# zhing2006/hala-renderer

Measured on AMD Instinct MI355X. Metric: Mrays/s, higher is better.
Workload: dtype f32

## Files before the change

hala-renderer_amd/csrc/renderer.hip:

```cpp
#include <hip/hip_runtime.h>

#include <algorithm>
#include <cmath>
#include <cstdio>
#include <cstring>
#include <memory>
#include <string>
#include <sys/stat.h>
#include <vector>

#include "adaptive.h"
#include "denoise.h"
#include "dyn_api.h"
#include "hala_types.h"
#include "host_image.h"
#include "host_scene.h"
#include "host_util.h"
#include "kernels.h"

namespace rt { std::string decode_image_file_rgba8(const char* path, uint32_t* w, uint32_t* h, std::vector<uint8_t>* rgba); }

using namespace rt;

namespace {
// ... 112 lines not shown
    std::vector<uint32_t> insts;
    DeviceArray<hala_gpu_mesh_data> d_md;
    DeviceArray<uint32_t> d_first, d_gid, d_inst;
    ~Blas() { if (b.topology) bvh_free_topology(b.topology); }
  };
  std::vector<std::unique_ptr<Blas>> blas;
  bool two_level = false;
  uint32_t instancing_mode = 0;
  std::vector<uint8_t> inst_instanced;
  std::vector<int32_t> prim_blas;
  uint32_t tlas_capacity = 0, tlas_nodes = 0, stored_tris = 0;
  std::vector<InstRef> inst_refs;
  DeviceArray<InstRef> d_inst_refs;
  DeviceArray<InstInfo> d_inst_info;
  DeviceArray<Tri> d_tris_by_id, d_tris;
  DeviceArray<Tri> d_tris_any;
  DeviceArray<ShadeTri> d_shade_tris;
  DeviceArray<BvhNode4> d_nodes;
  uint32_t lds_nodes = 0, lds_tris = 0;
  bool staged = false;
  uint32_t leaf_max_built = 0;
  float ray_eps = 0.0f;
  DeviceArray<uint2> d_spill;
  LaunchCfg lcfg{};
  uint32_t fuse_mode = 1;

  bool has_env = false;
  uint32_t env_w = 0, env_h = 0;
  DeviceArray<float4> d_env;
  DeviceArray<float> d_env_total, d_marginal, d_conditional;
  float env_total_sum = 0.0f;

  uint32_t real_pixels = 0;
  uint32_t rank = 0, world = 1, tile_size = 32, tiles_x = 0, tiles_y = 0, tiles_per_rank = 0, perm_a_inv = 0, perm_b = 7;
  uint32_t slot_count = 0;
  uint32_t blocks_x = 0;
  size_t image_pixels() const { return world <= 1 ? (size_t)width * height : (size_t)slot_count; }
  uint32_t batch_capacity = 1;

  DeviceArray<float4> img_local[4];
  DeviceArray<float4> img_full[4];
  bool full_valid[4] = {false, false, false, false};
  DenoiseBuffers denoise;
  bool denoised = false;
  AdaptiveState adaptive;
  DeviceArray<P3> ps_lr, ps_le, ps_alb, ps_nrm;
  DeviceArray<hala_ray> q_rays[2];
  DeviceArray<float4> q_state[2];
  DeviceArray<hala_hit> q_hits;
  DeviceArray<uint32_t> q_perm;
  DeviceArray<ShadowEntry> q_shadow[2];
  DeviceArray<Control> d_ctl;
  DeviceArray<WorkCounters> d_batch_work;

  uint64_t total_frames = 0;
  bool counting = false;
  hala_global_uniform last_uniform{};
  TraceEvents ring[kStatRing];
  int ring_pos = 0;
  bool vertices_dirty = false;
  bool materials_dirty_any = false;
  bool materials_dirty_any_refit = false;
  bool any_invisible = false;
  bool any_translucent = false;
  DeviceArray<uint8_t> d_material_any_class;
  std::vector<uint8_t> material_any_class;
  uint32_t launch_event_period = 0;
  unsigned long long update_counter = 0;
  hala_rt_statistics stats{};
  hipEvent_t scratch_event = nullptr;
  hipStream_t scratch_stream = nullptr;
  hipEvent_t batch_done = nullptr;
  ncclComm_t comm = nullptr;
  bool comm_owned = false;
  int comm_rank = 0, comm_world = 1;
  hipStream_t gather_stream = nullptr;
  DeviceArray<float4> gather_stage[4], gather_recv[4];
  hipEvent_t ev_rendered = nullptr, ev_staged = nullptr, ev_gathered = nullptr;
  uint32_t gather_pending = 0;
  int scratch_acquire(hipStream_t s) {
    if (scratch_event && scratch_stream != s) RT_HIP(hipStreamWaitEvent(s, scratch_event, 0));
    return HALA_OK;
  }

  ~hala_rt_renderer() {
    if (device >= 0) (void)hipSetDevice(device);
    if (stream) (void)hipStreamSynchronize(stream);
    for (auto& t : ring) {
      for (auto e : t.ev) (void)hipEventDestroy(e);
      if (t.frame_begin) (void)hipEventDestroy(t.frame_begin);
      if (t.frame_end) (void)hipEventDestroy(t.frame_end);
      if (t.host_totals) (void)hipHostFree(t.host_totals);
      if (t.host_sizes) (void)hipHostFree(t.host_sizes);
    }
    if (batch_done) (void)hipEventDestroy(batch_done);
    if (gather_stream) { (void)hipStreamSynchronize(gather_stream); (void)hipStreamDestroy(gather_stream); }
    for (hipEvent_t e : {ev_rendered, ev_staged, ev_gathered}) if (e) (void)hipEventDestroy(e);
    if (comm && comm_owned) { if (const RcclApi* api = rccl_api(nullptr)) (void)api->CommDestroy(comm); }
    for (auto& i : img_local) i.release();
    for (auto& i : img_full) i.release();
    if (bvh.topology) bvh_free_topology(bvh.topology);
    blas.clear();
    if (stream) (void)hipStreamDestroy(stream);
  }

  SceneView view() const {
    SceneView sv{};
    sv.nodes = d_nodes.ptr; sv.tris = d_tris.ptr; sv.tris_any = any_invisible ? d_tris_any.ptr : d_tris.ptr; sv.tris_by_id = d_tris_by_id.ptr; sv.shade_tris = d_shade_tris.ptr;
    sv.inst_first_tri = d_inst_first_tri.ptr; sv.primitives = d_instances.ptr; sv.materials = d_materials.ptr; sv.material_kind = d_material_kind.ptr;
    sv.lights = d_lights.ptr; sv.cameras = d_cameras.ptr;
    sv.textures = d_textures.ptr; sv.tex_arena = d_tex_arena.ptr; sv.tex_arena8 = d_tex_arena8.ptr; sv.tex_lut = d_srgb_lut.ptr; sv.texture_count = (uint32_t)host_textures.size(); sv.shade_sort = shade_sort ? 1u : 0u; sv.simple_materials = simple_materials ? 1u : 0u; sv.scatter_media = scatter_media ? 1u : 0u; sv.any_translucent = any_translucent ? 1u : 0u;
    sv.env_pixels = reinterpret_cast<const float*>(d_env.ptr); sv.env_marginal = d_marginal.ptr; sv.env_conditional = d_conditional.ptr;
    sv.node_count = bvh.node_count; sv.tri_count = bvh.tri_count; sv.lds_nodes = lds_nodes; sv.lds_tris = lds_tris;
    sv.inst_refs = d_inst_refs.ptr; sv.inst_info = d_inst_info.ptr; sv.instance_count = (uint32_t)hs.instances.size(); sv.two_level = two_level ? 1u : 0u;
    sv.ray_eps = ray_eps;
    sv.staged = staged ? 1u : 0u;
    return sv;
  }
  Queues queues() const {
    Queues q{};
    q.rays[0] = q_rays[0].ptr; q.rays[1] = q_rays[1].ptr; q.state[0] = q_state[0].ptr; q.state[1] = q_state[1].ptr;
    q.hits = q_hits.ptr; q.perm = q_perm.ptr; q.shadow[0] = q_shadow[0].ptr; q.shadow[1] = q_shadow[1].ptr;
    return q;
  }
  PathState path_state() const { return PathState{ps_lr.ptr, ps_le.ptr, ps_alb.ptr, ps_nrm.ptr}; }

  FrameConst frame_const(const hala_global_uniform& u, uint32_t samples = 1) const {
    FrameConst fc{};
    fc.u = u;
    fc.aspect = u.resolution[0] / u.resolution[1];
    float sn = 0.0f, cs = 1.0f;
    if (!hs.cameras.empty()) h_sincos_rad(0.5f * hs.cameras[0].yfov, &sn, &cs);
    fc.tan_half = sn / cs;
    fc.pixel_spread = 2.0f * fc.tan_half / u.resolution[1];
    fc.width = width; fc.height = height;
    fc.tile_size = tile_size; fc.tiles_x = tiles_x; fc.tiles_y = tiles_y; fc.world = world; fc.rank = rank; fc.blocks_x = blocks_x;
    fc.tiles_per_rank = tiles_per_rank; fc.perm_a = perm_a_inv; fc.perm_b = perm_b;
    fc.pixel_slots = slot_count; fc.samples = samples; fc.slot_count = slot_count * samples;
    if (adaptive.enabled) {
      fc.block_list = adaptive.lists[adaptive.cur].ptr;
      fc.pixel_slots = adaptive.active_blocks * kPixelBlock * kPixelBlock;
      fc.slot_count = fc.pixel_slots * samples;
    }
    return fc;
  }

  void reset_accumulation() {
    total_frames = 0;
    for (bool& v : full_valid) v = false;
    adaptive.restart(width * height);
  }
  uint32_t rendered_frames() const { return (uint32_t)std::min(total_frames, max_frames); }

  void resolve_slot(TraceEvents& t) {
    if (!t.pending) return;
    (void)hipEventSynchronize(t.frame_end);
    float ms = 0.0f;
    if (hipEventElapsedTime(&ms, t.frame_begin, t.frame_end) == hipSuccess) { stats.last_gpu_ms = ms; stats.gpu_ms_total += ms; }
    double tr[3] = {0.0, 0.0, 0.0}, sh = 0.0;
    unsigned long long rays[3] = {0, 0, 0}, launches[3] = {0, 0, 0};
    const QueueSizes* qs = t.host_sizes;
    for (size_t k = 0, depth = 0; k + 3 < t.used; k += 4, ++depth) {
      float m = 0.0f;
      const bool own_closest = depth == 0 || !((t.traced_mask >> depth) & 1ull);
      if (own_closest && hipEventElapsedTime(&m, t.ev[k], t.ev[k + 1]) == hipSuccess) {
        const unsigned long long n = depth == 0 ? (unsigned long long)t.primary_pixels * t.samples : qs->n_active[depth];
        tr[0] += m; rays[0] += n; launches[0] += 1;
        if (depth == 0) { stats.traverse_primary_ms_total += m; stats.traverse_primary_launches += 1; stats.rays_primary_timed += n; }
      }
      if (hipEventElapsedTime(&m, t.ev[k + 1], t.ev[k + 2]) == hipSuccess) sh += m;
      if (hipEventElapsedTime(&m, t.ev[k + 2], t.ev[k + 3]) == hipSuccess) {
        const unsigned long long ns = (unsigned long long)qs->n_shadow[0][depth] + qs->n_shadow[1][depth];
        if ((t.fused_mask >> depth) & 1ull) {
          tr[2] += m; launches[2] += 1;
          stats.rays_fused_shadow_timed += ns;
          if ((t.traced_mask >> (depth + 1)) & 1ull) stats.rays_fused_closest_timed += qs->n_active[depth + 1];
        } else { tr[1] += m; rays[1] += ns; }
      }
    }
    stats.traverse_ms_last_update = tr[0] + tr[1] + tr[2];
    stats.traverse_closest_ms_total += tr[0];
    stats.traverse_shadow_ms_total += tr[1];
    stats.traverse_fused_ms_total += tr[2];
    stats.shade_ms_total += sh;
    stats.traverse_closest_launches += launches[0];
    stats.traverse_fused_launches += launches[2];
    stats.shade_launches += t.used / 4;
    stats.traverse_shadow_launches += t.used ? t.shadow_launches : 0;
    stats.rays_closest_timed += rays[0]; stats.rays_shadow_timed += rays[1];
    stats.updates_rendered += t.samples;
    const Totals& tot = *t.host_totals;
    const unsigned long long rc = tot.rays_closest, rs = tot.rays_shadow;
    stats.rays_last_update = rc + rs;
    stats.rays_total += rc + rs;
    stats.rays_closest_total += rc;
    stats.rays_primary_total += (unsigned long long)t.primary_pixels * t.samples;
    stats.rays_shadow_total += rs;
    if (t.counted) {
      stats.nodes_closest_total += tot.steps[0][0]; stats.tris_closest_total += tot.steps[0][1];
      stats.nodes_shadow_total += tot.steps[1][0]; stats.tris_shadow_total += tot.steps[1][1];
      stats.rays_closest_counted += rc; stats.rays_shadow_counted += rs;
      stats.wave_steps_closest_total += tot.probe[0][0]; stats.leaf_passes_closest_total += tot.probe[0][1]; stats.leaf_lanes_closest_total += tot.probe[0][2];
      stats.nodes_primary_total += tot.primary_steps[0]; stats.tris_primary_total += tot.primary_steps[1];
      stats.rays_primary_counted += (unsigned long long)t.primary_pixels * t.samples;
      stats.wave_steps_shadow_total += tot.probe[1][0]; stats.leaf_passes_shadow_total += tot.probe[1][1]; stats.leaf_lanes_shadow_total += tot.probe[1][2];
    }
    t.pending = false;
  }
  hipEvent_t next_event(TraceEvents& t) {
    if (t.used == t.ev.size()) { hipEvent_t e = nullptr; (void)hipEventCreate(&e); t.ev.push_back(e); }
    return t.ev[t.used++];
  }
};

namespace {

int ensure_device(hala_rt_renderer* r) {
  if (!r) RT_FAIL("The renderer handle is null!");
  RT_HIP(hipSetDevice(r->device));
  return HALA_OK;
}

void compute_tiling(hala_rt_renderer* r) {
  if (r->world <= 1) {
    r->real_pixels = r->width * r->height;
    r->slot_count = r->real_pixels;
    r->blocks_x = 0;
    if (kPixelBlock) {
      r->blocks_x = (r->width + kPixelBlock - 1) / kPixelBlock;
      r->slot_count = r->blocks_x * ((r->height + kPixelBlock - 1) / kPixelBlock) * kPixelBlock * kPixelBlock;
    }
    r->tiles_x = r->tiles_y = r->tiles_per_rank = 0;
    return;
  }
  r->tiles_x = (r->width + r->tile_size - 1) / r->tile_size;
  r->tiles_y = (r->height + r->tile_size - 1) / r->tile_size;
  const uint32_t n = r->tiles_x * r->tiles_y;
  r->tiles_per_rank = (n + r->world - 1) / r->world;
  uint32_t A = 0x9E3779B1u % n;
  if (A == 0) A = 1;
  while (gcd_u32(A, n) != 1) ++A;
  r->perm_a_inv = mod_inverse(A, n);
  r->perm_b = 7;
  r->slot_count = r->tiles_per_rank * r->tile_size * r->tile_size;
  uint64_t real = 0;
  for (uint32_t t = 0; t < n; ++t) {
    const uint32_t k = (uint32_t)(((uint64_t)t * A + r->perm_b) % n);
    if (k % r->world != r->rank) continue;
    const uint32_t tx = t % r->tiles_x, ty = t / r->tiles_x;
    const uint32_t w = std::min(r->tile_size, r->width - tx * r->tile_size), h = std::min(r->tile_size, r->height - ty * r->tile_size);
    real += (uint64_t)w * h;
  }
  r->real_pixels = (uint32_t)real;
}

int alloc_wavefront(hala_rt_renderer* r, uint32_t samples) {
  const size_t n = (size_t)r->slot_count * samples;
  if (n > 0xfffffff0ull) RT_FAIL("The sample batch is too large for 32-bit path slots.");
  RT_HIP(r->ps_lr.resize(n)); RT_HIP(r->ps_le.resize(n)); RT_HIP(r->ps_alb.resize(n)); RT_HIP(r->ps_nrm.resize(n));
  RT_HIP(r->q_rays[0].resize(n)); RT_HIP(r->q_rays[1].resize(n)); RT_HIP(r->q_state[0].resize(n)); RT_HIP(r->q_state[1].resize(n));
  RT_HIP(r->q_hits.resize(n)); RT_HIP(r->q_perm.resize(n)); RT_HIP(r->q_shadow[0].resize(n)); RT_HIP(r->q_shadow[1].resize(n));
  r->batch_capacity = samples;
  return HALA_OK;
}

int alloc_frame_buffers(hala_rt_renderer* r) {
  const size_t n = r->slot_count;
  for (auto& i : r->img_local) { RT_HIP(i.resize(n)); RT_HIP(hipMemsetAsync(i.ptr, 0, n * sizeof(float4), r->stream)); }
  if (alloc_wavefront(r, 1) != HALA_OK) return HALA_ERR;
  RT_HIP(r->d_ctl.resize(1));
  RT_HIP(hipMemsetAsync(r->d_ctl.ptr, 0, sizeof(Control), r->stream));
  RT_HIP(r->d_batch_work.resize(1));
  return HALA_OK;
}

int upload_packed(hala_rt_renderer* r, bool geometry = true) {
  HostScene& hs = r->hs;
  if (geometry) {
  size_t nv = 0, ni = 0;
  r->prim_vertex_offset.clear(); r->prim_index_offset.clear();
  for (const auto& p : hs.prims) {
    r->prim_vertex_offset.push_back(nv); r->prim_index_offset.push_back(ni);
    nv += p.vertices.size();
    ni += (p.indices.size() + 3) & ~size_t(3);
  }
  RT_HIP(r->d_vertices.resize(nv)); RT_HIP(r->d_indices.resize(ni));
  for (size_t k = 0; k < hs.prims.size(); ++k) {
    const auto& p = hs.prims[k];
    if (!p.vertices.empty()) RT_HIP(hipMemcpyAsync(r->d_vertices.ptr + r->prim_vertex_offset[k], p.vertices.data(), p.vertices.size() * sizeof(hala_vertex), hipMemcpyHostToDevice, r->stream));
    if (!p.indices.empty()) RT_HIP(hipMemcpyAsync(r->d_indices.ptr + r->prim_index_offset[k], p.indices.data(), p.indices.size() * 4, hipMemcpyHostToDevice, r->stream));
  }
  }
  for (size_t i = 0; i < hs.instances.size(); ++i) {
    const uint32_t p = hs.instance_prim[i];
    hs.instances[i].vertices = reinterpret_cast<uint64_t>(r->d_vertices.ptr + r->prim_vertex_offset[p]);
    hs.instances[i].indices = reinterpret_cast<uint64_t>(r->d_indices.ptr + r->prim_index_offset[p]);
  }
  RT_HIP(r->d_cameras.upload(hs.cameras.data(), hs.cameras.size(), r->stream));
  RT_HIP(r->d_lights.upload(hs.lights.data(), hs.lights.size(), r->stream));
  RT_HIP(r->d_materials.upload(hs.gpu_materials.data(), hs.gpu_materials.size(), r->stream));
  {
    std::vector<uint8_t> kind(hs.gpu_materials.size());
    for (size_t i = 0; i < kind.size(); ++i) kind[i] = shade_kind_of(hs.gpu_materials[i], (uint32_t)hs.texture_image.size());
    RT_HIP(r->d_material_kind.upload(kind.data(), kind.size(), r->stream));
    r->material_kind = kind;
    uint32_t seen = 0;
    for (uint8_t k : kind) seen |= 1u << k;
    r->shade_sort = (seen & (seen - 1u)) != 0u;
    r->scatter_media = false;
    for (const auto& m : hs.gpu_materials) r->scatter_media = r->scatter_media || m.medium_type == 2u;
    r->simple_materials = seen == (1u << kShadeKindFirst);
  }
  RT_HIP(r->d_instances.upload(hs.instances.data(), hs.instances.size(), r->stream));
  RT_HIP(r->d_inst_first_tri.upload(hs.inst_first_tri.data(), hs.inst_first_tri.size(), r->stream));
  RT_HIP(hipStreamSynchronize(r->stream));
  return HALA_OK;
}

int upload_textures(hala_rt_renderer* r) {
  const HostScene& hs = r->hs;
  std::vector<TexDesc> img_desc(hs.images.size());
  size_t total_f = 0, total_8 = 0, largest_8 = 0;
  for (size_t k = 0; k < hs.images.size(); ++k) {
    TexDesc& td = img_desc[k];
    memset(&td, 0, sizeof(td));
    td.width = hs.images[k].width; td.height = hs.images[k].height; td.format = hs.images[k].format;
    uint32_t m = std::max(td.width, td.height), p2 = 1, lg = 0;
    while (p2 < m) { p2 <<= 1; ++lg; }
    td.mips = std::min<uint32_t>(lg + 1, kMaxMips);
    size_t& total = td.format == kTexFloat ? total_f : total_8;
    for (uint32_t l = 0; l < td.mips; ++l) {
      if (total > 0xffffffffull) RT_FAIL("The texture arena exceeds 2^32 texels.");
      td.mip_offset[l] = (uint32_t)total;
      const uint32_t lw = std::max(1u, td.width >> l), lh = std::max(1u, td.height >> l);
      total += td.format == kTexFloat ? (size_t)lw * lh : (size_t)tex_tiled_size(lw, lh);
    }
    if (td.format != kTexFloat) largest_8 = std::max(largest_8, (size_t)td.width * td.height);
  }
  RT_HIP(r->d_tex_arena.resize(total_f));
  RT_HIP(r->d_tex_arena8.resize(total_8));
  if (total_8) RT_HIP(hipMemsetAsync(r->d_tex_arena8.ptr, 0, total_8 * 4, r->stream));
  const float* lut = srgb_decode_lut();
  float thr[256];
  for (int k = 0; k < 255; ++k) thr[k] = (lut[k] + lut[k + 1]) * 0.5f;
  thr[255] = 3.402823466e+38f;
  float lut512[512];
  for (int k = 0; k < 256; ++k) { lut512[k] = lut[k]; lut512[256 + k] = (float)k / 255.0f; }
  RT_HIP(r->d_srgb_lut.upload(lut512, 512, r->stream));
  RT_HIP(r->d_srgb_thr.upload(thr, 256, r->stream));
  DeviceArray<uint32_t> staging;
  RT_HIP(staging.resize(largest_8));
  for (size_t k = 0; k < hs.images.size(); ++k) {
    const TexDesc& td = img_desc[k];
    if (td.format == kTexFloat) {
      RT_HIP(hipMemcpyAsync(r->d_tex_arena.ptr + td.mip_offset[0], hs.images[k].rgba.data(), (size_t)td.width * td.height * 16, hipMemcpyHostToDevice, r->stream));
      for (uint32_t l = 1; l < td.mips; ++l)
        launch_mip_downsample(r->d_tex_arena.ptr + td.mip_offset[l - 1], std::max(1u, td.width >> (l - 1)), std::max(1u, td.height >> (l - 1)),
                              r->d_tex_arena.ptr + td.mip_offset[l], std::max(1u, td.width >> l), std::max(1u, td.height >> l), r->stream);
    } else {
      RT_HIP(hipMemcpyAsync(staging.ptr, hs.images[k].rgba8.data(), (size_t)td.width * td.height * 4, hipMemcpyHostToDevice, r->stream));
      launch_tile8(staging.ptr, td.width, td.height, r->d_tex_arena8.ptr + td.mip_offset[0], r->stream);
      for (uint32_t l = 1; l < td.mips; ++l)
        launch_mip_downsample8(r->d_tex_arena8.ptr + td.mip_offset[l - 1], std::max(1u, td.width >> (l - 1)), std::max(1u, td.height >> (l - 1)),
                               r->d_tex_arena8.ptr + td.mip_offset[l], std::max(1u, td.width >> l), std::max(1u, td.height >> l), td.format,
                               r->d_srgb_lut.ptr, r->d_srgb_thr.ptr, r->stream);
    }
  }
  std::vector<TexDesc> tex(hs.texture_image.size());
  for (size_t i = 0; i < tex.size(); ++i) tex[i] = img_desc[hs.texture_image[i]];
  RT_HIP(r->d_textures.upload(tex.data(), tex.size(), r->stream));
  RT_HIP(hipStreamSynchronize(r->stream));
  RT_HIP(hipGetLastError());
  r->host_textures = tex;
  return HALA_OK;
}

int configure_traversal(hala_rt_renderer* r) {
  const size_t nb = (size_t)r->bvh.node_count * 64, tb = (size_t)r->bvh.tri_count * 48;
  r->staged = !r->two_level && nb + tb <= kLdsStageBudget;
  r->lds_nodes = r->staged ? r->bvh.node_count : 0u;
  r->lds_tris = r->staged ? r->bvh.tri_count : 0u;
  const TreeForm tree = tree_form(r->view());
  if (r->leaf_max_built > traverse_max_leaf(tree)) RT_FAIL("The BVH was built with larger leaves than the traversal variant for its size accepts.");
  const size_t smem = (size_t)r->lds_nodes * 64 + (size_t)r->lds_tris * 48 + traverse_fixed_lds_bytes(tree);
  const uint32_t per_cu = traverse_blocks_per_cu(smem, tree);
  if (per_cu == 0) RT_FAIL("The traversal kernel does not fit on a compute unit with the requested LDS staging.");
  r->lcfg.persistent_blocks = r->cu_count * std::min(per_cu, 8u);
  r->lcfg.smem = smem;
  r->lcfg.spill = nullptr;
  r->lcfg.refill = r->staged ? 64u : kRefillThreshold;
  if (r->two_level || r->bvh.stack_need > traverse_stack_lds_levels(tree)) {
    if (r->two_level || r->bvh.stack_need > traverse_stack_lds_levels(tree) + traverse_stack_spill_levels()) {
      std::vector<BvhNode4> nodes(r->bvh.node_count);
      RT_HIP(hipMemcpy(nodes.data(), r->d_nodes.ptr, nodes.size() * sizeof(BvhNode4), hipMemcpyDeviceToHost));
      std::vector<uint32_t> need(nodes.size(), 0u);
      for (size_t i = nodes.size(); i-- > 0;) {
        uint32_t inner = 0, deepest = 0;
        for (uint32_t ref : nodes[i].ref) {
          if (ref == kAbsent) continue;
          if (is_inst_leaf(ref)) {
            const uint32_t k = ref & 0x0fffffffu;
            ++inner;
            if (k < r->inst_refs.size() && r->inst_refs[k].root < need.size()) deepest = std::max(deepest, 4u + need[r->inst_refs[k].root]);
            continue;
          }
          if (ref & kLeafRef) continue;
          ++inner;
          if (ref < need.size()) deepest = std::max(deepest, need[ref]);
        }
        need[i] = inner ? inner - 1u + deepest : 0u;
      }
      r->bvh.stack_need = need.empty() ? 1u : std::max(1u, need[0]);
    }
    if (r->bvh.stack_need > traverse_stack_lds_levels(tree) + traverse_stack_spill_levels())
      RT_FAIL("The BVH is deeper than the traversal stack supports (" + std::to_string(r->bvh.max_depth) + " levels, " + std::to_string(r->bvh.stack_need) + " stack entries).");
    RT_HIP(r->d_spill.resize((size_t)r->lcfg.persistent_blocks * 256 * traverse_stack_spill_levels()));
    r->lcfg.spill = r->d_spill.ptr;
  }
  const float ex = r->bvh.scene_max[0] - r->bvh.scene_min[0], ey = r->bvh.scene_max[1] - r->bvh.scene_min[1], ez = r->bvh.scene_max[2] - r->bvh.scene_min[2];
  r->ray_eps = std::sqrt(std::fmaf(ez, ez, std::fmaf(ey, ey, ex * ex))) * 1e-5f;
  return HALA_OK;
}

int attach_any_triangles(hala_rt_renderer* r) {
  const HostScene& hs = r->hs;
  std::vector<uint8_t> cls(hs.gpu_materials.size());
  r->any_invisible = false; r->any_translucent = false;
  for (size_t i = 0; i < cls.size(); ++i) {
    const hala_gpu_material& m = hs.gpu_materials[i];
    const bool cutout = m.base_color_map_index < hs.texture_image.size() && hs.images[hs.texture_image[m.base_color_map_index]].has_alpha;
    cls[i] = any_class_of(m, cutout);
    r->any_invisible = r->any_invisible || cls[i] != 0;
    r->any_translucent = r->any_translucent || cls[i] >= 2;
  }
  r->material_any_class = cls;
  RT_HIP(r->d_material_any_class.upload(cls.data(), cls.size(), r->stream));
  if (r->any_invisible) RT_HIP(r->d_tris_any.resize(r->two_level ? r->stored_tris : r->hs.triangle_count));
  r->bvh.tris_any = r->any_invisible ? r->d_tris_any.ptr : nullptr;
  r->bvh.material_any_class = r->d_material_any_class.ptr;
  r->bvh.material_kind = r->d_material_kind.ptr;
  r->bvh.material_count = (uint32_t)r->hs.gpu_materials.size();
  return HALA_OK;
}

static float h_dot3(const float* a, const float* b) { return std::fmaf(a[2], b[2], std::fmaf(a[1], b[1], a[0] * b[0])); }
static void h_cross3(const float* a, const float* b, float* o) {
  o[0] = std::fmaf(a[1], b[2], -(a[2] * b[1])); o[1] = std::fmaf(a[2], b[0], -(a[0] * b[2])); o[2] = std::fmaf(a[0], b[1], -(a[1] * b[0]));
}
static bool world_to_object(const float* m, InstRef* o) {
  const float c0[3] = {m[0], m[1], m[2]}, c1[3] = {m[4], m[5], m[6]}, c2[3] = {m[8], m[9], m[10]};
  float k0[3], k1[3], k2[3];
  h_cross3(c1, c2, k0); h_cross3(c2, c0, k1); h_cross3(c0, c1, k2);
  const float det = h_dot3(c0, k0);
  if (!(det != 0.0f) || !std::isfinite(det)) return false;
  const float inv = 1.0f / det;
  for (int k = 0; k < 3; ++k) { o->r0[k] = k0[k] * inv; o->r1[k] = k1[k] * inv; o->r2[k] = k2[k] * inv; o->tr[k] = m[12 + k]; }
  for (int k = 0; k < 3; ++k)
    if (!std::isfinite(o->r0[k]) || !std::isfinite(o->r1[k]) || !std::isfinite(o->r2[k]) || !std::isfinite(o->tr[k])) return false;
  return true;
}
static void h_transform_point(const float* m, const float* p, float* o) {
  for (int k = 0; k < 3; ++k) o[k] = std::fmaf(m[8 + k], p[2], std::fmaf(m[4 + k], p[1], m[k] * p[0])) + m[12 + k];
}
static void classify_instances(hala_rt_renderer* r, std::vector<uint8_t>* flags) {
  const HostScene& hs = r->hs;
  flags->assign(hs.instances.size(), 0);
  constexpr uint32_t kFlattenLimit = 1u << 26;
  if (r->instancing_mode == 1u || (r->instancing_mode == 0u && hs.triangle_count <= kFlattenLimit)) return;
  std::vector<uint32_t> refs(hs.prims.size(), 0u);
  for (uint32_t p : hs.instance_prim) refs[p]++;
  for (size_t i = 0; i < hs.instances.size(); ++i) {
    InstRef tmp;
    (*flags)[i] = refs[hs.instance_prim[i]] >= 2u && hs.prims[hs.instance_prim[i]].indices.size() >= 3 && world_to_object(hs.instances[i].transform, &tmp) ? 1 : 0;
  }
}

int build_instance_levels(hala_rt_renderer* r) {
  const HostScene& hs = r->hs;
  std::vector<TlasItem> items;
  r->inst_refs.clear();
  std::vector<InstInfo> info(hs.instances.size());
  float smin[3] = {INFINITY, INFINITY, INFINITY}, smax[3] = {-INFINITY, -INFINITY, -INFINITY};
  uint32_t deepest = 0;
  std::vector<uint32_t> flat_base(hs.instances.size(), 0u);
  if (!r->blas.empty() && !r->blas[0]->object_space) {
    const hala_rt_renderer::Blas& w = *r->blas[0];
    uint32_t at = w.tri_off;
    for (uint32_t i : w.insts) { flat_base[i] = at; at += hs.inst_first_tri[i + 1] - hs.inst_first_tri[i]; }
    if (w.b.tri_count) {
      TlasItem it{};
      const float pad = std::max({std::fabs(w.b.scene_min[0]), std::fabs(w.b.scene_min[1]), std::fabs(w.b.scene_min[2]), std::fabs(w.b.scene_max[0]),
                                  std::fabs(w.b.scene_max[1]), std::fabs(w.b.scene_max[2])}) * 1.9073486328125e-06f * 2.0f;
      for (int k = 0; k < 3; ++k) { it.mn[k] = w.b.scene_min[k] - pad; it.mx[k] = w.b.scene_max[k] + pad; smin[k] = std::min(smin[k], w.b.scene_min[k]); smax[k] = std::max(smax[k], w.b.scene_max[k]); }
      it.ref = w.node_off;
      it.need = w.b.stack_need;
      deepest = std::max(deepest, w.b.max_depth);
      items.push_back(it);
    }
  }
// ... 144 lines not shown
  if (r->two_level) return build_two_level(r);
  const uint32_t n = r->hs.triangle_count;
  r->stored_tris = n; r->tlas_nodes = 0; r->tlas_capacity = 0;
  RT_HIP(r->d_tris_by_id.resize(n)); RT_HIP(r->d_tris.resize(n)); RT_HIP(r->d_shade_tris.resize(n));
  RT_HIP(r->d_nodes.resize(std::max<uint32_t>(n, 2) - 1));
  r->bvh.primitives = r->d_instances.ptr; r->bvh.inst_first_tri = r->d_inst_first_tri.ptr;
  r->bvh.instance_count = (uint32_t)r->hs.instances.size(); r->bvh.tri_count = n;
  r->bvh.tris_by_id = r->d_tris_by_id.ptr; r->bvh.shade_tris = r->d_shade_tris.ptr; r->bvh.tris = r->d_tris.ptr; r->bvh.nodes = r->d_nodes.ptr;
  if (attach_any_triangles(r) != HALA_OK) return HALA_ERR;
  uint32_t leaf_max = (size_t)n * 80 <= kLdsStageBudget ? kLeafMaxStaged : kLeafMax;
  if ((size_t)n * 80 > kLdsStageBudget) leaf_max = std::min(leaf_max, traverse_max_leaf(TreeForm::Large));
  const std::string e = bvh_build(r->bvh, leaf_max, r->stream);
  if (!e.empty()) RT_FAIL(e);
  r->leaf_max_built = leaf_max;
  return configure_traversal(r);
}

std::string file_stem(const char* path) {
  std::string p(path);
  const size_t slash = p.find_last_of("/\\");
  std::string base = slash == std::string::npos ? p : p.substr(slash + 1);
  const size_t dot = base.find_last_of('.');
  if (dot != std::string::npos && dot != 0) base = base.substr(0, dot);
  return base;
}

int install_envmap(hala_rt_renderer* r, const float* pixels, uint32_t channels, uint32_t w, uint32_t h, float rotation,
                   const float* cached_total, const float* cached_marginal, const float* cached_conditional) {
  if (!pixels || w == 0 || h == 0 || (channels != 3 && channels != 4)) RT_FAIL("Unsupported color type for environment map.");
  std::vector<float> data((size_t)w * h * 4);
  for (size_t i = 0; i < (size_t)w * h; ++i) {
    for (uint32_t c = 0; c < 3; ++c) {
      const float v = pixels[i * channels + c];
      if (std::isnan(v)) RT_FAIL("The pixel value is NaN!");
      if (std::isinf(v)) RT_FAIL("The pixel value is infinite!");
      data[4 * i + c] = v;
    }
    data[4 * i + 3] = 1.0f;
  }
  RT_HIP(r->d_env.upload(reinterpret_cast<const float4*>(data.data()), (size_t)w * h, r->stream));
  RT_HIP(r->d_env_total.resize(1)); RT_HIP(r->d_marginal.resize(h)); RT_HIP(r->d_conditional.resize((size_t)w * h));
  if (cached_total) {
    RT_HIP(hipMemcpyAsync(r->d_env_total.ptr, cached_total, 4, hipMemcpyHostToDevice, r->stream));
    RT_HIP(hipMemcpyAsync(r->d_marginal.ptr, cached_marginal, (size_t)h * 4, hipMemcpyHostToDevice, r->stream));
    RT_HIP(hipMemcpyAsync(r->d_conditional.ptr, cached_conditional, (size_t)w * h * 4, hipMemcpyHostToDevice, r->stream));
    RT_HIP(hipStreamSynchronize(r->stream));
    r->env_total_sum = *cached_total;
  } else {
    const std::string e = envmap_build_distribution(r->d_env.ptr, w, h, r->d_env_total.ptr, r->d_marginal.ptr, r->d_conditional.ptr, r->stream);
    if (!e.empty()) RT_FAIL(e);
    RT_HIP(hipMemcpy(&r->env_total_sum, r->d_env_total.ptr, 4, hipMemcpyDeviceToHost));
  }
  r->env_w = w; r->env_h = h; r->has_env = true; r->env_rotation = rotation;
  return HALA_OK;
}

}

extern "C" {

const char* hala_last_error_message(void) { return get_last_error(); }
const char* hala_version(void) { return "halart 0.1 (gfx950)"; }

int hala_rt_create(const char* name, uint32_t width, uint32_t height, int device_ordinal, uint32_t max_depth, uint32_t rr_depth,
                   int enable_tonemap, int enable_aces, int use_simple_aces, uint64_t max_frames, hala_rt_renderer** out) {
  if (!out) RT_FAIL("The output handle is null!");
  *out = nullptr;
  if (width == 0 || height == 0) RT_FAIL("The renderer resolution is zero!");
  if (max_depth == 0 || max_depth > kMaxDepth) RT_FAIL("max_depth must be in 1.." + std::to_string(kMaxDepth) + ".");
  int count = 0;
  if (hipGetDeviceCount(&count) != hipSuccess || count <= 0) RT_FAIL("No HIP device is available: libhalart has no CPU path.");
  if (device_ordinal < 0 || device_ordinal >= count) RT_FAIL("The requested device ordinal does not exist.");
  RT_HIP(hipSetDevice(device_ordinal));
  std::unique_ptr<hala_rt_renderer> r(new hala_rt_renderer());
  r->name = name ? name : "";
  r->width = width; r->height = height; r->device = device_ordinal;
  r->max_depth = max_depth; r->rr_depth = rr_depth;
  r->enable_tonemap = enable_tonemap != 0; r->enable_aces = enable_aces != 0; r->use_simple_aces = use_simple_aces != 0;
  r->max_frames = max_frames == 0 ? UINT64_MAX : max_frames;
  hipDeviceProp_t prop;
  RT_HIP(hipGetDeviceProperties(&prop, device_ordinal));
  r->cu_count = (uint32_t)prop.multiProcessorCount;
  RT_HIP(hipStreamCreateWithFlags(&r->stream, hipStreamNonBlocking));
  compute_tiling(r.get());
  if (alloc_frame_buffers(r.get()) != HALA_OK) return HALA_ERR;
  RT_HIP(hipStreamSynchronize(r->stream));
  *out = r.release();
  return HALA_OK;
}

void hala_rt_destroy(hala_rt_renderer* r) { delete r; }

int hala_rt_push_general_shader(hala_rt_renderer* r, const void* code, size_t code_size, int stage, const char*) {
  if (!r) RT_FAIL("The renderer handle is null!");
  if (!code || code_size == 0) RT_FAIL("The shader code is empty!");
  if (stage == 0) r->n_raygen++; else if (stage == 1) r->n_miss++; else if (stage == 2) r->n_callable++; else RT_FAIL("Invalid general shader stage.");
  return HALA_OK;
}
int hala_rt_push_general_shader_with_file(hala_rt_renderer* r, const char* file_path, int stage, const char* debug_name) {
  if (!r) RT_FAIL("The renderer handle is null!");
  struct stat st;
  if (!file_path || stat(file_path, &st) != 0) RT_FAIL(std::string("Failed to load shader file \"") + (file_path ? file_path : "") + "\".");
  static const char dummy = 0;
  return hala_rt_push_general_shader(r, &dummy, 1, stage, debug_name);
}
int hala_rt_push_hit_shaders(hala_rt_renderer* r, const void* ch, size_t chs, const void* ah, size_t ahs, const void* is, size_t iss, const char*) {
  if (!r) RT_FAIL("The renderer handle is null!");
  if ((!ch || !chs) && (!ah || !ahs) && (!is || !iss)) RT_FAIL("The hit shader group is empty!");
  r->n_hit++;
  return HALA_OK;
}
int hala_rt_push_hit_shaders_with_file(hala_rt_renderer* r, const char* ch, const char* ah, const char* is, const char*) {
  if (!r) RT_FAIL("The renderer handle is null!");
  struct stat st;
  for (const char* p : {ch, ah, is}) if (p && stat(p, &st) != 0) RT_FAIL(std::string("Failed to load shader file \"") + p + "\".");
  if (!ch && !ah && !is) RT_FAIL("The hit shader group is empty!");
  r->n_hit++;
  return HALA_OK;
}

int hala_rt_load_blue_noise_pixels(hala_rt_renderer* r, const uint8_t* rgba8, uint32_t width, uint32_t height);
int hala_rt_load_blue_noise_texture(hala_rt_renderer* r, const char* path) {
  if (!r) RT_FAIL("The renderer handle is null!");
  if (!path || !*path || file_stem(path).empty()) RT_FAIL("The file name is none!");
  uint32_t w = 0, h = 0;
  std::vector<uint8_t> px;
  std::string e;
  try { e = rt::decode_image_file_rgba8(path, &w, &h, &px); }
  catch (const std::exception& ex) { e = std::string("Failed to open image \"") + path + "\": " + ex.what(); }
  if (!e.empty()) RT_FAIL(e);
  return hala_rt_load_blue_noise_pixels(r, px.data(), w, h);
}
int hala_rt_load_blue_noise_pixels(hala_rt_renderer* r, const uint8_t* rgba8, uint32_t width, uint32_t height) {
  if (ensure_device(r) != HALA_OK) return HALA_ERR;
  if (!rgba8 || !width || !height) RT_FAIL("The blue noise texture is empty!");
  RT_HIP(r->blue_noise.upload(rgba8, (size_t)width * height * 4, r->stream));
  RT_HIP(hipStreamSynchronize(r->stream));
  r->blue_w = width; r->blue_h = height;
  return HALA_OK;
}

int hala_rt_set_scene(hala_rt_renderer* r, const hala_scene_desc* scene) {
  RtRange range("halart::set_scene");
  if (ensure_device(r) != HALA_OK) return HALA_ERR;
  RT_HIP(hipStreamSynchronize(r->stream));
  r->has_scene = false; r->committed = false;
  const std::string e = r->hs.assign(scene);
  if (!e.empty()) RT_FAIL(e);
  if (upload_packed(r) != HALA_OK) return HALA_ERR;
  if (upload_textures(r) != HALA_OK) return HALA_ERR;
  r->has_scene = true;
  return HALA_OK;
}

int hala_rt_set_envmap_pixels(hala_rt_renderer* r, const float* pixels, uint32_t channels, uint32_t width, uint32_t height, float rotation_degrees) {
  if (ensure_device(r) != HALA_OK) return HALA_ERR;
  RT_HIP(hipStreamSynchronize(r->stream));
  return install_envmap(r, pixels, channels, width, height, rotation_degrees, nullptr, nullptr, nullptr);
}

int hala_rt_set_envmap_file(hala_rt_renderer* r, const char* path, float rotation_degrees) {
  if (ensure_device(r) != HALA_OK) return HALA_ERR;
  if (!path || !*path) RT_FAIL("The file name is none!");
  HostImage img;
  const std::string e = load_float_image(path, &img);
  if (!e.empty()) RT_FAIL(e);
  RT_HIP(hipStreamSynchronize(r->stream));
  const std::string cache = "./out/" + file_stem(path) + ".dist_cache";
  const size_t W = img.width, H = img.height;
  std::vector<float> blob(1 + H + W * H);
  FILE* f = fopen(cache.c_str(), "rb");
  if (f) {
    const size_t got = fread(blob.data(), 4, blob.size(), f);
    fclose(f);
    if (got != blob.size()) RT_FAIL("Failed to read from file.");
    return install_envmap(r, img.pixels.data(), img.channels, img.width, img.height, rotation_degrees, &blob[0], &blob[1], &blob[1 + H]);
  }
  if (install_envmap(r, img.pixels.data(), img.channels, img.width, img.height, rotation_degrees, nullptr, nullptr, nullptr) != HALA_OK) return HALA_ERR;
  blob[0] = r->env_total_sum;
  RT_HIP(hipMemcpy(&blob[1], r->d_marginal.ptr, H * 4, hipMemcpyDeviceToHost));
  RT_HIP(hipMemcpy(&blob[1 + H], r->d_conditional.ptr, W * H * 4, hipMemcpyDeviceToHost));
  f = fopen(cache.c_str(), "wb");
  if (!f) RT_FAIL("Failed to create file \"" + cache + "\".");
  const size_t put = fwrite(blob.data(), 4, blob.size(), f);
  if (fclose(f) != 0 || put != blob.size()) RT_FAIL("Failed to write to file.");
  return HALA_OK;
}

void hala_rt_set_ground_color(hala_rt_renderer* r, const float rgba[4]) { if (r && rgba) memcpy(r->ground, rgba, 16); }
void hala_rt_set_sky_color(hala_rt_renderer* r, const float rgba[4]) { if (r && rgba) memcpy(r->sky, rgba, 16); }
void hala_rt_set_env_intensity(hala_rt_renderer* r, float v) { if (r) r->env_intensity = v; }
void hala_rt_set_exposure_value(hala_rt_renderer* r, float v) { if (r) r->exposure = v; }

int hala_rt_commit(hala_rt_renderer* r) {
  RtRange range("halart::commit");
  if (ensure_device(r) != HALA_OK) return HALA_ERR;
  if (!r->has_scene) RT_FAIL("The scene in GPU is none!");
  if (r->hs.cameras.empty()) RT_FAIL("The scene has no camera.");
  if (r->hs.instances.empty()) RT_FAIL("The scene has no mesh primitive.");
  if (build_bvh(r) != HALA_OK) return HALA_ERR;
  r->committed = true;
  r->reset_accumulation();
  return HALA_OK;
}

int hala_rt_set_build_options(hala_rt_renderer* r, const hala_rt_build_options* o) {
  if (!r) RT_FAIL("The renderer handle is null!");
  if (!o) RT_FAIL("The build options are null!");
  if (o->builder > 3u || o->ploc_tail > 2u || o->instancing > 2u) RT_FAIL("Invalid build options.");
  for (uint32_t v : o->reserved) if (v != 0u) RT_FAIL("Invalid build options (reserved fields must be 0).");
  r->instancing_mode = o->instancing;
  r->bvh.opt.builder = o->builder; r->bvh.opt.ploc_tail = o->ploc_tail;
  r->bvh.opt.ploc_look_every = o->ploc_look_every; r->bvh.opt.collapse_look_every = o->collapse_look_every;
  return HALA_OK;
}

static int update_impl(hala_rt_renderer* r, uint32_t frames) {
  RtRange range("halart::update");
  if (ensure_device(r) != HALA_OK) return HALA_ERR;
  if (!r->committed) RT_FAIL("The pipeline is none!");
  const uint64_t first = r->total_frames;
  r->total_frames += frames;
  if (first >= r->max_frames) return HALA_OK;
  const uint32_t samples = (uint32_t)std::min<uint64_t>(frames, r->max_frames - first);
  if (samples > r->batch_capacity) {
    RT_HIP(hipStreamSynchronize(r->stream));
    if (alloc_wavefront(r, samples) != HALA_OK) return HALA_ERR;
  }
  hala_global_uniform u{};
  memcpy(u.ground_color, r->ground, 16); memcpy(u.sky_color, r->sky, 16);
  u.resolution[0] = (float)r->width; u.resolution[1] = (float)r->height;
  u.max_depth = r->max_depth; u.rr_depth = r->rr_depth;
  u.frame_index = (uint32_t)first;
  u.camera_index = 0;
  u.env_type = r->has_env ? 1u : 0u;
  u.env_map_width = r->has_env ? r->env_w : 0; u.env_map_height = r->has_env ? r->env_h : 0;
  u.env_total_sum = r->has_env ? r->env_total_sum : 0.0f;
  u.env_rotation = r->env_rotation / 360.0f;
  u.env_intensity = r->env_intensity; u.exposure_value = r->exposure;
  u.enable_tonemap = r->enable_tonemap; u.enable_aces = r->enable_aces; u.use_simple_aces = r->use_simple_aces;
  u.num_of_lights = (uint32_t)r->hs.lights.size();
  r->last_uniform = u;
  r->last_uniform.frame_index = (uint32_t)(first + samples - 1);
  AdaptiveState& ad = r->adaptive;
  if (ad.enabled && first == 0 && adaptive_begin(ad, r->stream) != hipSuccess) RT_FAIL("hala_rt_update: the adaptive sampling state could not be reset.");
  if (ad.enabled && ad.active_blocks == 0) {
    for (int k = 0; k < kStatRing; ++k) r->resolve_slot(r->ring[(r->ring_pos + k) % kStatRing]);
    r->stats.rays_last_update = 0;
    return HALA_OK;
  }
  const uint32_t primary_pixels = ad.enabled ? ad.active_pixels : r->real_pixels;

  TraceEvents& te = r->ring[r->ring_pos];
  r->ring_pos = (r->ring_pos + 1) % kStatRing;
  r->resolve_slot(te);
  if (!te.frame_begin) { RT_HIP(hipEventCreate(&te.frame_begin)); RT_HIP(hipEventCreate(&te.frame_end)); RT_HIP(hipHostMalloc(reinterpret_cast<void**>(&te.host_totals), sizeof(Totals), hipHostMallocDefault)); }
  te.used = 0; te.counted = r->counting; te.shadow_launches = 0; te.fused_mask = 0; te.traced_mask = 0;

  te.samples = samples;
  te.primary_pixels = primary_pixels;
  const FrameConst fc = r->frame_const(u, samples);
  const SceneView sv = r->view();
  const Queues q = r->queues();
  const PathState ps = r->path_state();
  Control* ctl = r->d_ctl.ptr;
  hipStream_t s = r->stream;
  if (r->scratch_acquire(s) != HALA_OK) return HALA_ERR;
  RT_HIP(hipEventRecord(te.frame_begin, s));
  RT_HIP(hipMemsetAsync(ctl, 0, sizeof(Control), s));
  const bool timed = r->launch_event_period == 1u || (r->launch_event_period > 1u && (r->update_counter % r->launch_event_period) == 0u);
  r->update_counter++;
  const bool fuse = (r->fuse_mode == 2u || (r->fuse_mode == 1u && !timed)) && !r->counting && (u.num_of_lights > 0 || u.env_type == 1u);
  if (timed && !te.host_sizes) RT_HIP(hipHostMalloc(reinterpret_cast<void**>(&te.host_sizes), sizeof(QueueSizes), hipHostMallocDefault));
  bool traced = false;
  for (uint32_t depth = 0; depth < r->max_depth; ++depth) {
    if (timed) { hipEvent_t a = r->next_event(te); RT_HIP(hipEventRecord(a, s)); }
    if (depth == 0) {
      launch_trace_primary(r->lcfg, sv, fc, q.hits, &ctl->work_closest, ctl, primary_pixels * samples, r->counting, s);
      if (r->counting) RT_HIP(hipMemcpyAsync(ctl->totals.primary_steps, ctl->totals.steps[0], 16, hipMemcpyDeviceToDevice, s));
    }
    else if (!traced) launch_trace_batch(r->lcfg, sv, q.rays[depth & 1u], q.hits, &ctl->sizes.n_active[depth], 0, &ctl->work_closest, ctl, false, r->counting, true, s);
    traced = false;
    if (timed) { hipEvent_t b = r->next_event(te); RT_HIP(hipEventRecord(b, s)); }
    launch_shade(fc, sv, q, ps, ctl, depth, s);
    if (timed) { hipEvent_t c = r->next_event(te); RT_HIP(hipEventRecord(c, s)); }
    const uint32_t kinds = (u.num_of_lights > 0 ? 1u : 0u) | (u.env_type == 1u ? 2u : 0u);
    const bool last = depth + 1u >= r->max_depth;
    if (fuse && kinds && (!last || kinds == 3u) && launch_trace_shadow_then_batch(r->lcfg, sv, q, ps, ctl, depth, kinds, !last, s)) {
      traced = !last;
      if (timed) { te.fused_mask |= 1ull << depth; if (traced) te.traced_mask |= 1ull << (depth + 1u); }
    }
    else
      for (uint32_t kind = 0; kind < 2u; ++kind) {
        if (!((kinds >> kind) & 1u)) continue;
        launch_trace_shadow(r->lcfg, sv, q, ps, ctl, depth, kind, r->counting, s);
        te.shadow_launches += timed ? 1u : 0u;
      }
    if (timed) { hipEvent_t d = r->next_event(te); RT_HIP(hipEventRecord(d, s)); }
  }
  launch_resolve(fc, ps, r->img_local[0].ptr, r->img_local[1].ptr, r->img_local[2].ptr, r->img_local[3].ptr, s);
  RT_HIP(hipMemcpyAsync(te.host_totals, &ctl->totals, sizeof(Totals), hipMemcpyDeviceToHost, s));
  if (timed) RT_HIP(hipMemcpyAsync(te.host_sizes, &ctl->sizes, sizeof(QueueSizes), hipMemcpyDeviceToHost, s));
  RT_HIP(hipEventRecord(te.frame_end, s));
  r->scratch_event = te.frame_end; r->scratch_stream = s;
  RT_HIP(hipGetLastError());
  te.pending = true;
  for (bool& v : r->full_valid) v = false;
  const uint32_t n = (uint32_t)(first + samples);
  if (ad.enabled && n == ad.p.min_samples / 2u) {
    RT_HIP(hipMemcpyAsync(ad.snapshot.ptr, r->img_local[0].ptr, ad.snapshot.bytes(), hipMemcpyDeviceToDevice, s));
    ad.last_snapshot = n;
  }
  if (ad.enabled && adaptive_is_check(ad.p, n)) {
    RT_HIP(adaptive_enqueue_check(ad, r->img_local[0].ptr, r->width, r->height, r->blocks_x, r->exposure, n, s));
    RT_HIP(hipStreamSynchronize(s));
    adaptive_finish_check(ad, n);
  }
  return HALA_OK;
}

int hala_rt_update(hala_rt_renderer* r, double, uint32_t, uint32_t) { return update_impl(r, 1); }

int hala_rt_update_batch(hala_rt_renderer* r, uint32_t frames) {
  if (!r) RT_FAIL("The renderer handle is null!");
  while (frames > 0) {
    uint32_t chunk = std::min(frames, kMaxSampleBatch);
    if (r->adaptive.enabled && r->total_frames < r->max_frames)
      chunk = (uint32_t)std::min<uint64_t>(chunk, adaptive_frames_to_event(r->adaptive.p, r->total_frames));
    if (update_impl(r, chunk) != HALA_OK) return HALA_ERR;
    frames -= chunk;
  }
  return HALA_OK;
}

int hala_rt_render(hala_rt_renderer* r) {
  if (ensure_device(r) != HALA_OK) return HALA_ERR;
  if (r->total_frames > r->max_frames) return HALA_OK;
  const TraceEvents& before_last = r->ring[(r->ring_pos + kStatRing - 2) % kStatRing];
  if (before_last.pending && before_last.frame_end) RT_HIP(hipEventSynchronize(before_last.frame_end));
  return HALA_OK;
}
int hala_rt_wait_idle(hala_rt_renderer* r) {
  if (ensure_device(r) != HALA_OK) return HALA_ERR;
  RT_HIP(hipStreamSynchronize(r->stream));
  return HALA_OK;
}

int hala_rt_read_image(hala_rt_renderer* r, int which, float* dst) {
  if (ensure_device(r) != HALA_OK) return HALA_ERR;
  if (which < 0 || which > 3 || !dst) RT_FAIL("Invalid image selector.");
  RT_HIP(hipStreamSynchronize(r->stream));
  const size_t bytes = (size_t)r->width * r->height * sizeof(float4);
  if (r->world <= 1) { RT_HIP(hipMemcpy(dst, r->img_local[which].ptr, bytes, hipMemcpyDeviceToHost)); return HALA_OK; }
  if (!r->full_valid[which]) RT_FAIL("The frame is sharded across ranks: gather the tiles (hala_rt_scatter_gathered_tiles) before reading the image.");
  RT_HIP(hipMemcpy(dst, r->img_full[which].ptr, bytes, hipMemcpyDeviceToHost));
  return HALA_OK;
}

int hala_rt_save_images(hala_rt_renderer* r, const char* path) {
  RtRange range("halart::save_images");
  if (ensure_device(r) != HALA_OK) return HALA_ERR;
  if (!path || !*path) RT_FAIL("The file name is none!");
  std::string p(path);
  const size_t slash = p.find_last_of("/\\");
  const std::string dir = slash == std::string::npos ? "" : p.substr(0, slash + 1);
  const std::string stem = file_stem(path);
  std::vector<float> px((size_t)r->width * r->height * 4);
  static const char* suffix[3] = {"_color.pfm", "_albedo.pfm", "_normal.pfm"};
  for (int which = 0; which < 3; ++which) {
    if (hala_rt_read_image(r, which, px.data()) != HALA_OK) return HALA_ERR;
    if (which == 0) tonemap_pixels(px.data(), (size_t)r->width * r->height, r->enable_tonemap, r->enable_aces, r->use_simple_aces);
    const std::string e = write_pfm((dir + stem + suffix[which]).c_str(), px.data(), r->width, r->height);
    if (!e.empty()) RT_FAIL(e);
  }
  return HALA_OK;
}

int hala_rt_get_info(hala_rt_renderer* r, hala_rt_info* out) {
  if (!r || !out) RT_FAIL("The renderer handle is null!");
  out->width = r->width; out->height = r->height;
  return HALA_OK;
}
int hala_rt_get_statistics(hala_rt_renderer* r, hala_rt_statistics* out) {
  if (ensure_device(r) != HALA_OK) return HALA_ERR;
  if (!out) RT_FAIL("The output pointer is null!");
  RT_HIP(hipStreamSynchronize(r->stream));
  for (int k = 0; k < kStatRing; ++k) r->resolve_slot(r->ring[(r->ring_pos + k) % kStatRing]);
  r->stats.total_frames = r->total_frames;
  *out = r->stats;
  return HALA_OK;
}
int hala_rt_reset_accumulation(hala_rt_renderer* r) {
  if (!r) RT_FAIL("The renderer handle is null!");
  r->reset_accumulation();
  return HALA_OK;
}

int hala_rt_set_adaptive_sampling(hala_rt_renderer* r, const hala_adaptive_params* p) {
  if (p) {
    const std::string bad = adaptive_check_params(p);
    if (!bad.empty()) RT_FAIL(bad);
  }
  if (ensure_device(r) != HALA_OK) return HALA_ERR;
  AdaptiveState& ad = r->adaptive;
  if (p) {
    if (kPixelBlock != 8u) RT_FAIL("Adaptive sampling needs the 8 x 8 pixel blocks of RENDER_SPEC 9 (this build has RT_PIXEL_BLOCK = " + std::to_string(kPixelBlock) + ").");
    if (r->world > 1) RT_FAIL("Adaptive sampling is not available on a sharded renderer (world > 1).");
    if (!ad.enabled) {
      RT_HIP(hipStreamSynchronize(r->stream));
      const uint32_t blocks = r->blocks_x * ((r->height + kPixelBlock - 1) / kPixelBlock);
      RT_HIP(ad.ensure(blocks, (size_t)r->width * r->height));
    }
    ad.p = *p;
    ad.enabled = true;
  } else if (ad.enabled) {
    RT_HIP(hipStreamSynchronize(r->stream));
    ad.release();
    ad.enabled = false;
  }
// ... 706 lines not shown
```

Before: 5217.

## Overlap last-bounce shadow trace and resolve with next frame on a tail stream

Moves the final bounce's shadow tracing, the resolve and the totals readback onto a second stream, so the next update's primary trace can start while the previous frame's tail is still running. To make that safe it double-buffers the Control block, gives the tail stream its own traversal-stack spill buffer, and joins the tail stream before primary shading and at every read, sync or adaptive point. This adds cross-stream event bookkeeping and hazards on shared path-state buffers, and the overlap is limited because the join comes right after the next primary trace.

```diff
diff --git a/hala-renderer_amd/csrc/renderer.hip b/hala-renderer_amd/csrc/renderer.hip
--- a/hala-renderer_amd/csrc/renderer.hip
+++ b/hala-renderer_amd/csrc/renderer.hip
@@ -218,10 +218,22 @@
     if (scratch_event && scratch_stream != s) RT_HIP(hipStreamWaitEvent(s, scratch_event, 0));
     return HALA_OK;
   }
+  hipStream_t tail_stream = nullptr;
+  hipEvent_t ev_shaded = nullptr;
+  hipEvent_t tail_done = nullptr;
+  bool tail_open = false;
+  uint32_t ctl_pos = 0;
+  DeviceArray<uint2> d_spill_tail;
+  int join_tail() {
+    if (tail_open) RT_HIP(hipStreamWaitEvent(stream, tail_done, 0));
+    tail_open = false;
+    return HALA_OK;
+  }
 
   ~hala_rt_renderer() {
     if (device >= 0) (void)hipSetDevice(device);
     if (stream) (void)hipStreamSynchronize(stream);
+    if (tail_stream) (void)hipStreamSynchronize(tail_stream);
     for (auto& t : ring) {
       for (auto e : t.ev) (void)hipEventDestroy(e);
       if (t.frame_begin) (void)hipEventDestroy(t.frame_begin);
@@ -237,6 +249,8 @@
     for (auto& i : img_full) i.release();
     if (bvh.topology) bvh_free_topology(bvh.topology);
     blas.clear();
+    if (ev_shaded) (void)hipEventDestroy(ev_shaded);
+    if (tail_stream) (void)hipStreamDestroy(tail_stream);
     if (stream) (void)hipStreamDestroy(stream);
   }
 
@@ -351,9 +365,10 @@
 
 namespace {
 
-int ensure_device(hala_rt_renderer* r) {
+int ensure_device(hala_rt_renderer* r, bool join = true) {
   if (!r) RT_FAIL("The renderer handle is null!");
   RT_HIP(hipSetDevice(r->device));
+  if (join && r->join_tail() != HALA_OK) return HALA_ERR;
   return HALA_OK;
 }
 
@@ -404,8 +419,8 @@
   const size_t n = r->slot_count;
   for (auto& i : r->img_local) { RT_HIP(i.resize(n)); RT_HIP(hipMemsetAsync(i.ptr, 0, n * sizeof(float4), r->stream)); }
   if (alloc_wavefront(r, 1) != HALA_OK) return HALA_ERR;
-  RT_HIP(r->d_ctl.resize(1));
-  RT_HIP(hipMemsetAsync(r->d_ctl.ptr, 0, sizeof(Control), r->stream));
+  RT_HIP(r->d_ctl.resize(2));
+  RT_HIP(hipMemsetAsync(r->d_ctl.ptr, 0, 2 * sizeof(Control), r->stream));
   RT_HIP(r->d_batch_work.resize(1));
   return HALA_OK;
 }
@@ -551,6 +566,7 @@
     if (r->bvh.stack_need > traverse_stack_lds_levels(tree) + traverse_stack_spill_levels())
       RT_FAIL("The BVH is deeper than the traversal stack supports (" + std::to_string(r->bvh.max_depth) + " levels, " + std::to_string(r->bvh.stack_need) + " stack entries).");
     RT_HIP(r->d_spill.resize((size_t)r->lcfg.persistent_blocks * 256 * traverse_stack_spill_levels()));
+    RT_HIP(r->d_spill_tail.resize(r->d_spill.count));
     r->lcfg.spill = r->d_spill.ptr;
   }
   const float ex = r->bvh.scene_max[0] - r->bvh.scene_min[0], ey = r->bvh.scene_max[1] - r->bvh.scene_min[1], ez = r->bvh.scene_max[2] - r->bvh.scene_min[2];
@@ -861,6 +877,8 @@
   RT_HIP(hipGetDeviceProperties(&prop, device_ordinal));
   r->cu_count = (uint32_t)prop.multiProcessorCount;
   RT_HIP(hipStreamCreateWithFlags(&r->stream, hipStreamNonBlocking));
+  RT_HIP(hipStreamCreateWithFlags(&r->tail_stream, hipStreamNonBlocking));
+  RT_HIP(hipEventCreateWithFlags(&r->ev_shaded, hipEventDisableTiming));
   compute_tiling(r.get());
   if (alloc_frame_buffers(r.get()) != HALA_OK) return HALA_ERR;
   RT_HIP(hipStreamSynchronize(r->stream));
@@ -996,13 +1014,14 @@
 
 static int update_impl(hala_rt_renderer* r, uint32_t frames) {
   RtRange range("halart::update");
-  if (ensure_device(r) != HALA_OK) return HALA_ERR;
+  if (ensure_device(r, false) != HALA_OK) return HALA_ERR;
   if (!r->committed) RT_FAIL("The pipeline is none!");
   const uint64_t first = r->total_frames;
   r->total_frames += frames;
   if (first >= r->max_frames) return HALA_OK;
   const uint32_t samples = (uint32_t)std::min<uint64_t>(frames, r->max_frames - first);
   if (samples > r->batch_capacity) {
+    if (r->join_tail() != HALA_OK) return HALA_ERR;
     RT_HIP(hipStreamSynchronize(r->stream));
     if (alloc_wavefront(r, samples) != HALA_OK) return HALA_ERR;
   }
@@ -1022,7 +1041,7 @@
   r->last_uniform = u;
   r->last_uniform.frame_index = (uint32_t)(first + samples - 1);
   AdaptiveState& ad = r->adaptive;
-  if (ad.enabled && first == 0 && adaptive_begin(ad, r->stream) != hipSuccess) RT_FAIL("hala_rt_update: the adaptive sampling state could not be reset.");
+  if (ad.enabled && first == 0 && (r->join_tail() != HALA_OK || adaptive_begin(ad, r->stream) != hipSuccess)) RT_FAIL("hala_rt_update: the adaptive sampling state could not be reset.");
   if (ad.enabled && ad.active_blocks == 0) {
     for (int k = 0; k < kStatRing; ++k) r->resolve_slot(r->ring[(r->ring_pos + k) % kStatRing]);
     r->stats.rays_last_update = 0;
@@ -1042,21 +1061,27 @@
   const SceneView sv = r->view();
   const Queues q = r->queues();
   const PathState ps = r->path_state();
-  Control* ctl = r->d_ctl.ptr;
-  hipStream_t s = r->stream;
-  if (r->scratch_acquire(s) != HALA_OK) return HALA_ERR;
+  Control* ctl = r->d_ctl.ptr + r->ctl_pos;
+  r->ctl_pos ^= 1u;
+  const hipStream_t s = r->stream;
+  const bool timed = r->launch_event_period == 1u || (r->launch_event_period > 1u && (r->update_counter % r->launch_event_period) == 0u);
+  r->update_counter++;
+  const bool split_tail = !timed && !r->counting;
+  if (!split_tail && r->join_tail() != HALA_OK) return HALA_ERR;
+  if (!r->tail_open && r->scratch_acquire(s) != HALA_OK) return HALA_ERR;
   RT_HIP(hipEventRecord(te.frame_begin, s));
   RT_HIP(hipMemsetAsync(ctl, 0, sizeof(Control), s));
-  const bool timed = r->launch_event_period == 1u || (r->launch_event_period > 1u && (r->update_counter % r->launch_event_period) == 0u);
-  r->update_counter++;
   const bool fuse = (r->fuse_mode == 2u || (r->fuse_mode == 1u && !timed)) && !r->counting && (u.num_of_lights > 0 || u.env_type == 1u);
   if (timed && !te.host_sizes) RT_HIP(hipHostMalloc(reinterpret_cast<void**>(&te.host_sizes), sizeof(QueueSizes), hipHostMallocDefault));
   bool traced = false;
+  hipStream_t ts = s;
+  LaunchCfg lc = r->lcfg;
   for (uint32_t depth = 0; depth < r->max_depth; ++depth) {
     if (timed) { hipEvent_t a = r->next_event(te); RT_HIP(hipEventRecord(a, s)); }
     if (depth == 0) {
       launch_trace_primary(r->lcfg, sv, fc, q.hits, &ctl->work_closest, ctl, primary_pixels * samples, r->counting, s);
       if (r->counting) RT_HIP(hipMemcpyAsync(ctl->totals.primary_steps, ctl->totals.steps[0], 16, hipMemcpyDeviceToDevice, s));
+      if (r->join_tail() != HALA_OK) return HALA_ERR;
     }
     else if (!traced) launch_trace_batch(r->lcfg, sv, q.rays[depth & 1u], q.hits, &ctl->sizes.n_active[depth], 0, &ctl->work_closest, ctl, false, r->counting, true, s);
     traced = false;
@@ -1065,27 +1090,35 @@
     if (timed) { hipEvent_t c = r->next_event(te); RT_HIP(hipEventRecord(c, s)); }
     const uint32_t kinds = (u.num_of_lights > 0 ? 1u : 0u) | (u.env_type == 1u ? 2u : 0u);
     const bool last = depth + 1u >= r->max_depth;
-    if (fuse && kinds && (!last || kinds == 3u) && launch_trace_shadow_then_batch(r->lcfg, sv, q, ps, ctl, depth, kinds, !last, s)) {
+    if (last && split_tail) {
+      RT_HIP(hipEventRecord(r->ev_shaded, s));
+      RT_HIP(hipStreamWaitEvent(r->tail_stream, r->ev_shaded, 0));
+      ts = r->tail_stream;
+      lc.spill = r->lcfg.spill ? r->d_spill_tail.ptr : nullptr;
+    }
+    if (fuse && kinds && (!last || kinds == 3u) && launch_trace_shadow_then_batch(lc, sv, q, ps, ctl, depth, kinds, !last, ts)) {
       traced = !last;
       if (timed) { te.fused_mask |= 1ull << depth; if (traced) te.traced_mask |= 1ull << (depth + 1u); }
     }
     else
       for (uint32_t kind = 0; kind < 2u; ++kind) {
         if (!((kinds >> kind) & 1u)) continue;
-        launch_trace_shadow(r->lcfg, sv, q, ps, ctl, depth, kind, r->counting, s);
+        launch_trace_shadow(lc, sv, q, ps, ctl, depth, kind, r->counting, ts);
         te.shadow_launches += timed ? 1u : 0u;
       }
     if (timed) { hipEvent_t d = r->next_event(te); RT_HIP(hipEventRecord(d, s)); }
   }
-  launch_resolve(fc, ps, r->img_local[0].ptr, r->img_local[1].ptr, r->img_local[2].ptr, r->img_local[3].ptr, s);
-  RT_HIP(hipMemcpyAsync(te.host_totals, &ctl->totals, sizeof(Totals), hipMemcpyDeviceToHost, s));
-  if (timed) RT_HIP(hipMemcpyAsync(te.host_sizes, &ctl->sizes, sizeof(QueueSizes), hipMemcpyDeviceToHost, s));
-  RT_HIP(hipEventRecord(te.frame_end, s));
-  r->scratch_event = te.frame_end; r->scratch_stream = s;
+  launch_resolve(fc, ps, r->img_local[0].ptr, r->img_local[1].ptr, r->img_local[2].ptr, r->img_local[3].ptr, ts);
+  RT_HIP(hipMemcpyAsync(te.host_totals, &ctl->totals, sizeof(Totals), hipMemcpyDeviceToHost, ts));
+  if (timed) RT_HIP(hipMemcpyAsync(te.host_sizes, &ctl->sizes, sizeof(QueueSizes), hipMemcpyDeviceToHost, ts));
+  RT_HIP(hipEventRecord(te.frame_end, ts));
+  r->scratch_event = te.frame_end; r->scratch_stream = ts;
+  r->tail_done = te.frame_end; r->tail_open = ts != s;
   RT_HIP(hipGetLastError());
   te.pending = true;
   for (bool& v : r->full_valid) v = false;
   const uint32_t n = (uint32_t)(first + samples);
+  if (ad.enabled && (n == ad.p.min_samples / 2u || adaptive_is_check(ad.p, n)) && r->join_tail() != HALA_OK) return HALA_ERR;
   if (ad.enabled && n == ad.p.min_samples / 2u) {
     RT_HIP(hipMemcpyAsync(ad.snapshot.ptr, r->img_local[0].ptr, ad.snapshot.bytes(), hipMemcpyDeviceToDevice, s));
     ad.last_snapshot = n;
@@ -1113,7 +1146,7 @@
 }
 
 int hala_rt_render(hala_rt_renderer* r) {
-  if (ensure_device(r) != HALA_OK) return HALA_ERR;
+  if (ensure_device(r, false) != HALA_OK) return HALA_ERR;
   if (r->total_frames > r->max_frames) return HALA_OK;
   const TraceEvents& before_last = r->ring[(r->ring_pos + kStatRing - 2) % kStatRing];
   if (before_last.pending && before_last.frame_end) RT_HIP(hipEventSynchronize(before_last.frame_end));
```

Result: faster. 5305, median of 6 (+1.7%).
